# TGoldC/Motion-Planning-for-Autonomous-Driving-with-MPC

Hardware: AMD Instinct MI355X
Metric: MPC steps/sec (N=30, nx=6 nu=2) at batch=4096 (higher is better)
Workload: dtype f64; 1 GPU; N=30 nx=6 nu=2 bicycle lane-following, batch=4096/GPU, tol 1e-8; mode=converged, gpu=AMD Radeon Graphics

## Files before the change

motion-planning-for-autonomous-driving-with-mpc_amd/csrc/mpc_stamps.h:

```cpp
#pragma once
#include <algorithm>
#include <cstdarg>
#include <cstdio>
#include <string>
#include <vector>

namespace mpc {
constexpr int STAMP_SLOTS = 16;
#define MPC_STAMP(dbg, row, slot, pred) do { if ((dbg) && (pred)) (dbg)[(row) * STAMP_SLOTS + (slot)] = __builtin_amdgcn_s_memtime(); } while (0)

enum StageStamp { SB_ENTER, SB_ISSUED, SB_LOADED, SB_P1, SB_RED1, SB_LS, SB_UPDATE, SB_XCHG, SB_EVAL, SB_RED3, SB_END };
enum RicStamp { RT_BEGIN, RT_BWD_END, RT_FWD_END, RT_B15_WAIT, RT_B15_GO, RT_B15_END, RT_F15_WAIT, RT_F15_GO, RT_F15_END, RT_F0 };
enum PipeStamp { PW_TAKE = 11, PW_GOT, PW_BCAST, PW_DONE, PW_SIGNALLED,
                 PR_WAIT = 11, PR_SWEEP, PR_PUBLISHED };
enum WgStamp { WG_ROUND = 12, WG_RECORDS, WG_SWEPT, WG_ROUND_END };
enum StartStamp { PP_BOUNDS = 1, PP_DEFECTS, PP_SCAN1, PP_SCAN2, PP_SCAN3, PP_SUMS,
                  KS_BEGIN = 11, KS_ROWS, KS_STORED, KS_SAFE, KS_FENCED };

struct StampSpan { int from, to; const char* label; };
constexpr StampSpan START_SPANS[] = {
    {KS_BEGIN, KS_ROWS, "rows->LDS"}, {KS_ROWS, KS_STORED, "Z/REF stores"}, {KS_STORED, PP_BOUNDS, "bounds+a0"}, {PP_BOUNDS, PP_DEFECTS, "defects"}, {PP_DEFECTS, PP_SCAN1, "scan1"},
    {PP_SCAN1, PP_SCAN2, "tan+scan2"}, {PP_SCAN2, PP_SCAN3, "sincos+scan3"}, {PP_SCAN3, PP_SUMS, "ROLL+sums"}, {PP_SUMS, KS_SAFE, "decide"}, {KS_SAFE, KS_FENCED, "fence"},
    {KS_FENCED, SB_ENTER, "enter"}, {SB_ENTER, SB_XCHG, "init point+exchange"}, {SB_XCHG, SB_EVAL, "eval+assemble"}, {SB_EVAL, SB_RED3, "reduce"}, {SB_RED3, SB_END, "finish"}};
constexpr StampSpan WG_SPANS[] = {
    {WG_ROUND, WG_RECORDS, "records"}, {WG_RECORDS, WG_SWEPT, "sweeps"}, {WG_SWEPT, SB_ENTER, "enter"}, {SB_ENTER, SB_ISSUED, "load+premath"}, {SB_ISSUED, SB_LOADED, "or"}, {SB_LOADED, SB_P1, "P1"},
    {SB_P1, SB_RED1, "reduce1+ls-begin"}, {SB_RED1, SB_LS, "linesearch"}, {SB_LS, SB_UPDATE, "P3-update"}, {SB_UPDATE, SB_XCHG, "exchange"}, {SB_XCHG, SB_EVAL, "P4-eval"},
    {SB_EVAL, SB_RED3, "reduce3"}, {SB_RED3, SB_END, "P5"}, {SB_END, WG_ROUND_END, "drain"}};
constexpr StampSpan STAGE_SPANS[] = {
    {SB_ENTER, SB_ISSUED, "issue-loads"}, {SB_ISSUED, SB_LOADED, "wait+barrier"}, {SB_LOADED, SB_P1, "P1"}, {SB_P1, SB_RED1, "reduce1"}, {SB_RED1, SB_LS, "linesearch"},
    {SB_LS, SB_UPDATE, "P3-update"}, {SB_UPDATE, SB_XCHG, "exchange"}, {SB_XCHG, SB_EVAL, "P4-eval"}, {SB_EVAL, SB_RED3, "reduce3"}, {SB_RED3, SB_END, "P5"}};
constexpr StampSpan PIPE_STAGE_SPANS[] = {
    {PW_TAKE, PW_GOT, "dequeue"}, {PW_GOT, PW_BCAST, "acquire+bcast"}, {PW_BCAST, SB_ENTER, "enter"}, STAGE_SPANS[0], STAGE_SPANS[1], STAGE_SPANS[2], STAGE_SPANS[3], STAGE_SPANS[4], STAGE_SPANS[5],
    STAGE_SPANS[6], STAGE_SPANS[7], STAGE_SPANS[8], STAGE_SPANS[9], {SB_END, PW_DONE, "drain"}, {PW_DONE, PW_SIGNALLED, "signal"}};
constexpr StampSpan PIPE_RIC_SPANS[] = {
    {PR_WAIT, PR_SWEEP, "wait"}, {PR_SWEEP, RT_BWD_END, "backward"}, {RT_BWD_END, RT_FWD_END, "forward"}, {RT_FWD_END, PR_PUBLISHED, "publish"}, {RT_B15_WAIT, RT_B15_GO, "barrier"},
    {RT_B15_GO, RT_B15_END, "step"}, {RT_F15_WAIT, RT_F15_GO, "barrier"}, {RT_F15_GO, RT_F15_END, "step"}, {RT_BWD_END, RT_F0, "first forward stage"}};
constexpr StampSpan RIC_SPANS[] = {
    {RT_BEGIN, RT_BWD_END, "backward"}, {RT_BWD_END, RT_FWD_END, "forward"}, {RT_B15_WAIT, RT_B15_GO, "bwd barrier-wait"}, {RT_B15_GO, RT_B15_END, "compute"},
    {RT_F15_WAIT, RT_F15_GO, "fwd barrier-wait"}, {RT_F15_GO, RT_F15_END, "compute"}};

inline void appendf(std::string& s, const char* fmt, ...) {
    char buf[512];
    va_list ap;
    va_start(ap, fmt);
    vsnprintf(buf, sizeof buf, fmt, ap);
    va_end(ap);
    s += buf;
}
template <bool WRAP = false, size_t N, class Ran>
int span_sums(const unsigned long long* rows, int nrows, const StampSpan (&sp)[N], double (&acc)[N], Ran ran) {
    int cnt = 0;
    for (double& a : acc) a = 0.0;
    for (const unsigned long long* r = rows; r < rows + (size_t)nrows * STAMP_SLOTS; r += STAMP_SLOTS) {
        if (!ran(r)) continue;
        for (size_t q = 0; q < N; ++q) acc[q] += WRAP ? (double)(r[sp[q].to] - r[sp[q].from]) : (double)(long long)(r[sp[q].to] - r[sp[q].from]);
        ++cnt;
    }
    return cnt;
}
template <bool WRAP = false, size_t N, class Ran>
std::string span_means(const char* head, const unsigned long long* rows, int nrows, const StampSpan (&sp)[N], Ran ran) {
    double acc[N];
    const int cnt = span_sums<WRAP>(rows, nrows, sp, acc, ran);
    std::string s;
    appendf(s, head, cnt);
    for (size_t q = 0; q < N; ++q) appendf(s, " %s=%.0f", sp[q].label, cnt ? acc[q] / cnt : 0.0);
    return s;
}
inline std::string format_start_timing(const unsigned long long* rows, int nblk) {
    unsigned long long t0 = ~0ull, t1 = 0ull;
    for (int b = 0; b < nblk; ++b) { t0 = std::min(t0, rows[b * STAMP_SLOTS + KS_BEGIN]); t1 = std::max(t1, rows[b * STAMP_SLOTS + SB_END]); }
    std::string s = span_means("[mpcgpu k_start timing, shader-clock ticks, mean over %d workgroups]", rows, nblk, START_SPANS, [](const unsigned long long*) { return true; });
    appendf(s, "; first start to last end %.0f\n", (double)(t1 - t0));
    return s;
}
inline std::string format_wg_timing(const unsigned long long* rows, int nblk) {
    return span_means("[mpcgpu k_solve_wg timing, shader-clock ticks, third round of %d workgroups]", rows, nblk, WG_SPANS,
                      [](const unsigned long long* r) { return r[WG_ROUND_END] && r[SB_END]; }) + "\n";
}
inline std::string format_pipe_timing(const unsigned long long* rows, int n_wg) {
    auto stage = [](const unsigned long long* r) { return r[PW_SIGNALLED] && r[SB_END]; };
    std::string s = span_means("[mpcgpu pipeline timing, shader-clock ticks, last item of %d stage workers]", rows, n_wg, PIPE_STAGE_SPANS, stage);
    double ra[9];
    const int nr = span_sums(rows, n_wg, PIPE_RIC_SPANS, ra, [&](const unsigned long long* r) { return !stage(r) && r[PR_PUBLISHED] && r[RT_FWD_END]; });
    for (double& v : ra) v = nr ? v / nr : 0.0;
    appendf(s, "\n[last pass of %d Riccati workers] wait=%.0f backward=%.0f forward=%.0f publish=%.0f; stage 15 of the backward sweep: barrier=%.0f step=%.0f, of the forward sweep: barrier=%.0f step=%.0f, its first stage starts %.0f ticks after the backward sweep\n",
            nr, ra[0], ra[1], ra[2], ra[3], ra[4], ra[5], ra[6], ra[7], ra[8]);
    return s;
}
inline std::string format_stage_timing(const unsigned long long* rows, int nblk, int ntiles) {
    std::string s = span_means<true>("[mpcgpu stage timing, shader-clock ticks per block, mean over %d blocks]", rows, nblk, STAGE_SPANS,
                                     [](const unsigned long long* r) { return r[SB_END] != 0; }) + "\n";
    const unsigned long long* rr = rows + (size_t)8 * nblk;
    const int nt = std::min(ntiles, nblk / 2);
    auto ran = [](const unsigned long long* r) { return r[RT_FWD_END] != 0; };
    auto tile0 = [&](int q) { return (long long)(rr[RIC_SPANS[q].to] - rr[RIC_SPANS[q].from]); };
    if (nt > 0 && ran(rr))
        appendf(s, "[riccati stage 15 of tile 0] bwd barrier-wait=%lld compute=%lld | fwd barrier-wait=%lld compute=%lld\n", tile0(2), tile0(3), tile0(4), tile0(5));
    double ric[6];
    const int c2 = span_sums<true>(rr, nt, RIC_SPANS, ric, ran);
    appendf(s, "[mpcgpu riccati timing, ticks per workgroup, mean over %d] backward=%.0f forward=%.0f\n", c2, c2 ? ric[0] / c2 : 0.0, c2 ? ric[1] / c2 : 0.0);
    return s;
}
inline std::string format_wg_trace(const unsigned long long* hw, int n_wtrace) {
    unsigned long long t0 = ~0ull, t1 = 0ull;
    std::vector<int> live;
    for (int w = 0; w < n_wtrace; ++w) if (hw[4 * w + 2]) { t0 = std::min(t0, hw[4 * w]); t1 = std::max(t1, hw[4 * w + 1]); live.push_back(w); }
    std::string s;
    if (live.empty()) return s;
    std::sort(live.begin(), live.end(), [&](int a, int b) { return hw[4 * a + 1] > hw[4 * b + 1]; });
    int late = 0;
    double start_max = 0;
    for (int w : live) { const double st = (double)(hw[4 * w] - t0) * 1e-2; if (st > 5.0) ++late; start_max = std::max(start_max, st); }
    appendf(s, "[mpcgpu wg_trace] %d workgroups with work of %d; span %.1f us; %d of them start more than 5 us after the first (latest start %.1f us); the last to finish:\n",
            (int)live.size(), n_wtrace, (double)(t1 - t0) * 1e-2, late, start_max);
    for (size_t i = 0; i < live.size() && i < 12; ++i) {
        const int w = live[i];
        const double st = (double)(hw[4 * w] - t0) * 1e-2, en = (double)(hw[4 * w + 1] - t0) * 1e-2;
        const double tf = (double)((hw[4 * w + 3] >> 16) & 0xFFFFFFull) * 1e-2, tr1 = (double)((hw[4 * w + 3] >> 40) & 0xFFFFFFull) * 1e-2;
        appendf(s, "    workgroup %5d: start %6.1f us  end %6.1f us  rounds %2d  instance-rounds %2d  -> %.1f us per round; instances taken over after %.1f us, first round done after %.1f us, later rounds %.1f us each\n",
                w, st, en, (int)hw[4 * w + 2], (int)(hw[4 * w + 3] & 0xFFFFu), (en - st) / (double)hw[4 * w + 2], tf, tr1, hw[4 * w + 2] > 1 ? (en - st - tr1) / (double)(hw[4 * w + 2] - 1) : 0.0);
    }
    return s;
}

}
```

motion-planning-for-autonomous-driving-with-mpc_amd/csrc/mpcgpu.hip:

```cpp
#include <hip/hip_runtime.h>
#include <type_traits>

#include <algorithm>
#include <cctype>
#include <cstdio>
#include <cstdlib>
#include <cstring>
#include <new>
#include <string>
#include <vector>

#include "mpc_host_common.h"
#include "mpc_solve_plan.h"
#include "mpc_stamps.h"
#include "mpc_closed_loop.h"
#include "mpc_forces_qp.h"
#include "mpc_riccati_mfma.h"
#include "mpc_sens.h"
#include "mpc_loop_lin.h"

using namespace mpc;

namespace {

// ... 860 lines not shown
    }
    if (A.ho_list != nullptr && t < 64 && pipe_ld(abort_w) == 0u) {
        pipe_acquire();
        asm volatile("s_waitcnt vmcnt(0)" ::: "memory");
        for (;;) {
            uint32_t j = 0u;
            if (t == 0) j = pipe_add(X + PX_HO_TICKET, 1u);
            j = (uint32_t)__builtin_amdgcn_readfirstlane((int)j);
            if (j >= n_tiles_x) break;
            ho_lists(P, (j * n_xcd + xcd) * 64u + (uint32_t)t, A.ho_list, A.ctl + PIPE_HO, stage_done);
        }
    }
    if (t == 0) {
        unsigned long long* st = reinterpret_cast<unsigned long long*>(A.ctl + PIPE_STATS);
        atomicAdd(st + P64_STAGE_WAIT, waited);
        atomicAdd(st + P64_STAGE_BUSY, busy + wall_clock64());
        atomicAdd(st + P64_ITEMS, (unsigned long long)n_items);
        pipe_add(abort_w + PH_STAGE_WORKERS, 1u);
    }
#endif
}

struct PrestartFromWs {
    __device__ __forceinline__ double z(int, int, int) const { return 0.0; }
    __device__ __forceinline__ double ref0(int, int) const { return 0.0; }
};
template <int NX, class Src = PrestartFromWs> __device__ __forceinline__ void prestart_par_block(const PRef& P, const uint32_t b0, double* sm, const Src src = Src{});

template <int NX, bool OSTG = false>
__device__ __attribute__((noinline)) void wg_restart(const PRef& Pin, const int n_mult, const int n_z, const int stash_rows, const uint32_t b0, double* lds,
                                                     uint32_t* live_out, const bool carry, const bool from_xs, const bool keep_first, const bool first_tiled) {
    const PRef P = mpc_pref(static_cast<const Params&>(Pin), false);
    using D = Dim<NX>;
    const int t = threadIdx.x, N = P.N, bx = P.bx;
    struct { int b, k, mb, bl; } c;
    c.k = t / bx;
    c.bl = t & (bx - 1);
    c.mb = (int)blockIdx.x * bx;
    c.b = (int)b0 + c.bl;
    const bool valid = (c.k <= N) && (c.b < P.B);
    if (valid) {
        constexpr int NZ = D::NZ;
        double v[MPC_EV(NZ)];
        static_assert(2 * MPC_EV(NZ) <= D::NPK, "two iterates fit the cost-to-go rows of a stage");
        if (keep_first) {
            if (first_tiled) ws_load_rows<NZ>(MPC_ROWS(MPC_K(P.Z, NZ, 0, e)), v);
            else ws_load_rows<NZ>(MPC_ROWS(MPC_KI(P.MZ, NZ, 0, e)), v);
            ws_store_rows<NZ>(MPC_ROWS(MPC_K(P.PK, D::NPK, 0, MPC_EV(NZ) + e)), v);
            if (c.k == 0) MPC_S(P.SC, SC_E0S) = (double)MPC_S(P.SC, SC_E0);
        }
        if (carry) {
            ws_load_rows<NZ>(MPC_ROWS(MPC_KI(P.MZ, NZ, 0, e)), v);
            ws_store_rows<NZ>(MPC_ROWS(MPC_K(P.PK, D::NPK, 0, e)), v);
        }
        if (from_xs) {
            if (!carry) ws_load_rows<NZ>(MPC_ROWS(MPC_K(P.PK, D::NPK, 0, e)), v);
        } else {
            const size_t nw = (size_t)2 * N + (size_t)NX * (N + 1);
            const double* xr = P.x0 + (size_t)c.b * nw;
            v[0] = (c.k < N) ? MPC_GP(xr, 2 * c.k) : 0.0;
            v[1] = (c.k < N) ? MPC_GP(xr, 2 * c.k + 1) : 0.0;
#pragma unroll
            for (int i = 0; i < NX; ++i) v[2 + i] = MPC_GP(xr, 2 * N + NX * c.k + i);
        }
        ws_store_rows<NZ>(MPC_ROWS(MPC_K(P.Z, NZ, 0, e)), v);
    }
    asm volatile("s_waitcnt vmcnt(0)" ::: "memory");
    lds_barrier();
    __builtin_amdgcn_fence(__ATOMIC_ACQ_REL, "workgroup");
    asm volatile("s_waitcnt vmcnt(0)" ::: "memory");
    prestart_par_block<NX>(P, b0, lds);
    asm volatile("s_waitcnt vmcnt(0)" ::: "memory");
    lds_barrier();
    __builtin_amdgcn_fence(__ATOMIC_ACQ_REL, "workgroup");
    asm volatile("s_waitcnt vmcnt(0)" ::: "memory");
    stage_block<NX, true, 256, 0xFFu, NoStepWait, OSTG>(P, n_mult, n_z, stash_rows, b0, ~0ull, lds, false, live_out);
    asm volatile("s_waitcnt vmcnt(0)" ::: "memory");
    lds_barrier();
    __builtin_amdgcn_fence(__ATOMIC_ACQ_REL, "workgroup");
    asm volatile("s_waitcnt vmcnt(0)" ::: "memory");
}

template <int NX>
__device__ __attribute__((noinline)) void wg_restore_first(const PRef& Pin, const uint32_t b0, const int st0, const int it0) {
    const PRef P = mpc_pref(static_cast<const Params&>(Pin), false);
    using D = Dim<NX>;
    constexpr int NZ = D::NZ;
    const int t = threadIdx.x, bx = P.bx;
    struct { int b, k, mb, bl; } c;
    c.k = t / bx;
    c.bl = t & (bx - 1);
    c.mb = (int)blockIdx.x * bx;
    c.b = (int)b0 + c.bl;
    if (c.k <= P.N && c.b < P.B) {
        double v[MPC_EV(NZ)];
        ws_load_rows<NZ>(MPC_ROWS(MPC_K(P.PK, D::NPK, 0, MPC_EV(NZ) + e)), v);
        ws_store_rows<NZ>(MPC_ROWS(MPC_KI(P.MZ, NZ, 0, e)), v);
        ws_store_rows<NZ>(MPC_ROWS(MPC_K(P.Z, NZ, 0, e)), v);
        if (c.k == 0) {
            MPC_S(P.SC, SC_E0) = (double)MPC_S(P.SC, SC_E0S);
            MPC_S(P.ISC, IS_STATUS) = st0;
            MPC_S(P.ISC, IS_ITERS) = it0;
        }
    }
    asm volatile("s_waitcnt vmcnt(0)" ::: "memory");
    lds_barrier();
    __builtin_amdgcn_fence(__ATOMIC_ACQ_REL, "workgroup");
    asm volatile("s_waitcnt vmcnt(0)" ::: "memory");
}

struct WgRescue { double ol_raw, relax; int32_t on; };
constexpr int RESC_LEVELS = 8;
__device__ __forceinline__ double resc_fraction(int q) { return q == 2 || q == 7 ? 1.0 : q == 4 ? 0.4 : q == 5 ? 0.7 : q == 6 ? 0.9 : 0.0; }
__device__ __forceinline__ bool resc_last(int q) { return q == 2 || q == 7; }

#if defined(__HIP_DEVICE_COMPILE__)
typedef const __attribute__((address_space(4))) Params* mpc_kernarg_params;
__device__ __forceinline__ mpc_kernarg_params wg_kernarg() {
    mpc_kernarg_params kp = (mpc_kernarg_params)__builtin_amdgcn_kernarg_segment_ptr();
    asm volatile("" : "+s"(kp));
    return kp;
}
__device__ __forceinline__ EmitDst wg_emit_dst() {
    const mpc_kernarg_params kp = wg_kernarg();
    return EmitDst{kp->x_out, kp->status_out, kp->iters_out, kp->kkt_out, kp->fail_count};
}
#else
inline EmitDst wg_emit_dst() { return EmitDst{}; }
#endif
template <int NX, int VAR, bool RESC>
__device__ __forceinline__ void solve_wg_body(const Params& Pk, const int n_mult, const int n_z, const int stash_rows, uint32_t* stats, const uint32_t* skip_if,
                                              const WgRescue& resc, unsigned long long* wtrace, const int32_t* list, const uint32_t* list_n) {
    PRef P(Pk);
#if defined(__HIP_DEVICE_COMPILE__)
    const bool emit_exit = RESC && resc.on && Pk.emit != 0;
    if (RESC && emit_exit) P.emit = 0;
    extern __shared__ __attribute__((aligned(16))) double lds[];
    __shared__ uint32_t sh_mask;
    __shared__ int sh_next[2];
    if (skip_if != nullptr && *skip_if != 0u) return;
    const double tol0 = P.tol;
    bool fresh = true;
    using D = Dim<NX>;
    using RC = Rec<NX>;
    const int bx = P.bx, t = threadIdx.x, N = P.N;
    const int lane = t;
    const uint32_t b0 = (blockIdx.x + (uint32_t)P.tile0 * (64u / (uint32_t)bx)) * (uint32_t)bx;
    int ib0 = (int)b0 < P.B ? (int)b0 : -1, ib1 = (bx > 1 && (int)b0 + 1 < P.B) ? (int)b0 + 1 : -1;
    uint32_t in_mb = 0u;
    if (list != nullptr) {
        uint32_t cnt[HO_BUCKETS], n = 0u;
#pragma unroll
        for (int q = 0; q < (int)HO_BUCKETS; ++q) { cnt[q] = list_n[q]; n += cnt[q]; }
        auto entry = [&](uint32_t v) -> int {
            if (v >= n) return -1;
#pragma unroll
            for (int q = 0; q < (int)HO_BUCKETS; ++q) { if (v < cnt[q]) return list[(uint32_t)q * (uint32_t)P.Bp + v]; v -= cnt[q]; }
            return -1;
        };
        const uint32_t G = gridDim.x;
        ib0 = lds_uniform(entry(blockIdx.x));
        ib1 = bx > 1 ? lds_uniform(entry(2u * G - 1u - blockIdx.x)) : -1;
        if (ib0 < 0) return;
        in_mb = ((ib0 & HO_IN_MB) ? 1u : 0u) | ((ib1 >= 0 && (ib1 & HO_IN_MB)) ? 2u : 0u);
        ib0 &= ~HO_IN_MB;
        if (ib1 >= 0) ib1 &= ~HO_IN_MB;
    }
    struct { int b, k, mb, bl; } c;
    c.k = t / bx;
    c.bl = t & (bx - 1);
    c.mb = (int)blockIdx.x * bx;
    c.b = c.bl ? ib1 : ib0;
    const bool valid = (c.k <= N) && (c.b >= 0) && (c.b < P.B);
    const mpc_lds_ptr recs = (mpc_lds_ptr)(lds_ptr_t)lds + WgLds<NX>::PAD;
    const mpc_lds_ptr dump = (mpc_lds_ptr)(lds_ptr_t)lds;
    double* const lds_bnd = lds + WgLds<NX>::PAD + (size_t)RC::SIZE * ((N + 1) * bx);
    double* const lds_c0 = lds_bnd + 2 * (N + 1) * D::NZ;
    double* const lds_r0 = lds_c0 + 8 * bx;
    double* const lds_rn = lds_r0 + 8 * bx;
    double* const lds_scl = lds_rn + 64 * NX;
    bool bounds_ok = false;
    double dl0 = 0.0, dl1 = 0.0;
    WgIo io{0u, 0u, lds_c0, lds_rn, lds_r0, lds_scl, true, false};
    const MfmaWords lane_words = mfma_lane_load<NX>(lane);
    uint32_t rounds = 0, sweeps = 0, inst_rounds = 0, prev_mask = 0u;
    const unsigned long long t_begin = wtrace ? wall_clock64() : 0ull;
    unsigned long long t_fresh = 0ull, t_round1 = 0ull;
    if (RESC && resc.on && t == 0 && ib0 >= 0 && ib0 < P.B) MPC_UB(P.ISC, (uint32_t)IS_RLEV, ib0) = 0;
    for (;;) {
        if (rounds == 0u && t < 64) {
            const int bb = t ? ib1 : ib0;
            const bool run = t < bx && bb >= 0 && bb < P.B && (list != nullptr || (int32_t)MPC_UB(P.ISC, (uint32_t)IS_STATUS, bb >= 0 ? bb : 0) == ST_RUNNING);
            const unsigned long long mk = __ballot(run ? 1 : 0);
            if (t == 0) sh_mask = (uint32_t)mk;
        }
        lds_barrier();
        const uint32_t mask = lds_uniform(sh_mask);
        if (Pk.emit != 0 && !emit_exit) {
            const uint32_t gone = prev_mask & ~mask;
            if (gone != 0u && valid && ((gone >> c.bl) & 1u)) {
                double z[MPC_EV(D::NZ)];
                ws_load_rows<D::NZ>(MPC_ROWS(MPC_KI(P.MZ, D::NZ, 0, e)), z);
                int st = 0, it = 0;
                double e0 = 0.0;
                if (c.k == 0) { st = (int32_t)MPC_S(P.ISC, IS_STATUS); it = (int32_t)MPC_S(P.ISC, IS_ITERS); e0 = MPC_S(P.SC, SC_E0); }
                emit_row<NX>(wg_emit_dst(), N, c.b, c.k, z, st, it, e0);
            }
            prev_mask = mask;
        }
        if (mask == 0u) {
            if (!RESC || !resc.on) break;
            if (t == 0) {
                const int bb = ib0;
                int next = -1, carry = 0;
                if (bb >= 0 && bb < P.B) {
                    const int st = (int32_t)MPC_UB(P.ISC, (uint32_t)IS_STATUS, bb), it = (int32_t)MPC_UB(P.ISC, (uint32_t)IS_ITERS, bb);
                    const int lev = (int32_t)MPC_UB(P.ISC, (uint32_t)IS_RLEV, bb);
                    const int q = lev & 0xFF;
                    int has_xs = (lev >> 8) & 1, first = lev & ~0x1FF;
                    int acc = (q == 0 ? 0 : (int32_t)MPC_UB(P.ISC, (uint32_t)IS_ITACC, bb)) + it;
                    if (q == 0) {
                        if (st == 0 || st == -7) { next = 1; first = (st == -7 ? 0x200 : 0) | (it << 16); if (stats != nullptr) atomicAdd(stats + WGS_RESCUED, 1u); }
                    } else {
                        if (st == 1) { carry = 1; has_xs = 1; }
                        if (!resc_last(q)) next = q + 1;
                        else if (st != 1 && q == 2) { next = 3; has_xs = 0; acc = first >> 16; }
                    }
                    if (next >= 0) {
                        MPC_UB(P.ISC, (uint32_t)IS_RLEV, bb) = next | (has_xs << 8) | first;
                        MPC_UB(P.ISC, (uint32_t)IS_ITACC, bb) = acc;
                        next |= has_xs << 8;
                    } else if (q != 0) {
                        if (st == 1) MPC_UB(P.ISC, (uint32_t)IS_ITERS, bb) = acc;
                        else next = -2 - ((first >> 9) & 1) - 2 * (first >> 16);
                    }
                }
                sh_next[0] = next;
                sh_next[1] = carry;
            }
            lds_barrier();
            const int nx_lev = lds_uniform(sh_next[0]), carry = lds_uniform(sh_next[1]);
            lds_barrier();
            if (nx_lev <= -2) {
                const int code = -2 - nx_lev;
                const PRef Pc = P;
                wg_restore_first<NX>(Pc, (uint32_t)ib0, (code & 1) ? -7 : 0, code >> 1);
            }
            if (nx_lev < 0) break;
            const int q = nx_lev & 0xFF;
            const bool from_xs = (nx_lev >> 8) != 0;
            {
                const double lo = resc_fraction(q) * resc.ol_raw;
                P.ol = lo - resc.relax * fmax(1.0, fabs(lo));
                P.tol = resc_last(q) ? tol0 : fmax(tol0, 1e-4);
            }
            {
                const PRef Pc = P;
                if (VAR == 2 || Pc.per_inst_obst != OBST_PER_STAGE) wg_restart<NX>(Pc, n_mult, n_z, stash_rows, (uint32_t)ib0, lds, &sh_mask, carry != 0, from_xs, q == 1, rounds == 0u);
                else wg_restart<NX, true>(Pc, n_mult, n_z, stash_rows, (uint32_t)ib0, lds, &sh_mask, carry != 0, from_xs, q == 1, rounds == 0u);
            }
            fresh = true;
            bounds_ok = false;
            io.have = false;
            continue;
        }
        ++rounds;
        inst_rounds += (uint32_t)__popc(mask);
        MPC_STAMP(P.DBG, blockIdx.x, WG_ROUND, t == 0 && rounds == 3u);
        const bool by_pipe = !RESC && valid && ((in_mb >> c.bl) & 1u) != 0u;
        if (fresh && valid && !by_pipe) {
            auto move = [&](auto cnt, auto from, auto to) {
                constexpr int CNT = decltype(cnt)::value;
                double v[MPC_EV(CNT)];
                ws_load_rows<CNT>(from, v);
                ws_store_rows<CNT>(to, v);
            };
            constexpr int NZ = D::NZ;
            move(std::integral_constant<int, NZ>{}, MPC_ROWS(MPC_K(P.Z, NZ, 0, e)), MPC_ROWS(MPC_KI(P.MZ, NZ, 0, e)));
            move(std::integral_constant<int, NZ>{}, MPC_ROWS(MPC_K(P.ZL, NZ, 0, e)), MPC_ROWS(MPC_KI(P.MZL, NZ, 0, e)));
            move(std::integral_constant<int, NZ>{}, MPC_ROWS(MPC_K(P.ZU, NZ, 0, e)), MPC_ROWS(MPC_KI(P.MZU, NZ, 0, e)));
            move(std::integral_constant<int, 4>{}, MPC_ROWS(MPC_K(P.SO, 3, 0, e)), MPC_ROWS(MPC_KI(P.MSO, 3, 0, e)));
            move(std::integral_constant<int, 4>{}, MPC_ROWS(MPC_K(P.NUO, 3, 0, e)), MPC_ROWS(MPC_KI(P.MNUO, 3, 0, e)));
            move(std::integral_constant<int, 4>{}, MPC_ROWS(MPC_K(P.ZLO, 3, 0, e)), MPC_ROWS(MPC_KI(P.MZLO, 3, 0, e)));
            move(std::integral_constant<int, 4>{}, MPC_ROWS(MPC_K(P.ZUO, 3, 0, e)), MPC_ROWS(MPC_KI(P.MZUO, 3, 0, e)));
            move(std::integral_constant<int, NX>{}, MPC_ROWS(MPC_K(P.LAM, NX, 0, e)), MPC_ROWS(MPC_KI(P.MLAM, NX, 0, e)));
        }
        if (fresh) {
            asm volatile("s_waitcnt vmcnt(0)" ::: "memory");
            __builtin_amdgcn_fence(__ATOMIC_ACQ_REL, "workgroup");
            asm volatile("s_waitcnt vmcnt(0)" ::: "memory");
        }
        const bool whole = fresh, tiled = fresh && !by_pipe;
        auto build_records = [&]() {
            if (valid && ((mask >> (t & (bx - 1))) & 1u)) {
                double blk[MPC_EV(D::NBLK)];
                if (tiled) ws_load_rows<D::NBLK>(MPC_ROWS(MPC_K(P.BLK, D::NBLK, 0, e)), blk);
                else ws_load_rows<D::NBLK>(MPC_ROWS(MPC_KI(P.MBLK, D::NBLK, 0, e)), blk);
                double hx0 = 0.0, hx1 = 0.0;
                if (c.k == 0) { hx0 = MPC_S(P.SC, SC_HUX0); hx1 = MPC_S(P.SC, SC_HUX1); }
                const mpc_lds_ptr r = recs + ((t & (bx - 1)) * (N + 1) + c.k) * RC::SIZE;
#pragma unroll
                for (int i = 0; i < D::NBLK; ++i) {
                    const bool kept = i < D::B_RUU || (i >= D::B_CN && i < D::B_CN + NX);
                    if (whole || !kept) r[RC::slot(i)] = (i >= D::B_CN && i < D::B_CN + NX) ? -blk[i] : blk[i];
                }
                r[RC::ZERO] = 0.0;
                r[RC::ONE] = 1.0;
                r[RC::DT] = P.dt;
                r[RC::HX] = hx0;
                r[RC::HX + 1] = hx1;
            }
        };
        if (fresh) {
            build_records();
            const int a0 = ib0 >= 0 ? ib0 : 0, a1 = ib1 >= 0 ? ib1 : a0;
            dl0 = lds_uniform((double)MPC_UB(P.SC, (uint32_t)SC_DLAST, a0));
            dl1 = lds_uniform((double)MPC_UB(P.SC, (uint32_t)SC_DLAST, a1));
            io.ill = ((int32_t)MPC_UB(P.ISC, (uint32_t)IS_ILL, a0) != 0 ? 1u : 0u) | ((bx > 1 && (int32_t)MPC_UB(P.ISC, (uint32_t)IS_ILL, a1) != 0) ? 2u : 0u);
            if (valid && c.k == 0) {
#pragma unroll
                for (int i = 0; i < NX; ++i) lds_c0[(t & (bx - 1)) * 8 + i] = MPC_S(P.SC, SC_C0 + i);
                double* q = lds_scl + c.bl * WgScl::SIZE;
                q[WgScl::MU] = MPC_S(P.SC, SC_MU); q[WgScl::TAU] = MPC_S(P.SC, SC_TAU); q[WgScl::DF] = MPC_S(P.SC, SC_DF); q[WgScl::THETA] = MPC_S(P.SC, SC_THETA);
                q[WgScl::FCOST] = MPC_S(P.SC, SC_FCOST); q[WgScl::LOGSUM] = MPC_S(P.SC, SC_LOGSUM); q[WgScl::THMAX] = MPC_S(P.SC, SC_THMAX);
                q[WgScl::THMIN] = MPC_S(P.SC, SC_THMIN); q[WgScl::A0LB] = MPC_S(P.SC, SC_A0LB); q[WgScl::A0UB] = MPC_S(P.SC, SC_A0UB);
                q[WgScl::STATUS] = (double)(int32_t)MPC_S(P.ISC, IS_STATUS); q[WgScl::NFILT] = (double)(int32_t)MPC_S(P.ISC, IS_NFILT);
                q[WgScl::ITERS] = (double)(int32_t)MPC_S(P.ISC, IS_ITERS); q[WgScl::CONV] = (double)(int32_t)MPC_S(P.ISC, IS_CONV);
                q[WgScl::FROW] = (double)(int32_t)MPC_S(P.ISC, IS_FROW); q[WgScl::HAVETH0] = (double)(int32_t)MPC_S(P.ISC, IS_HAVETH0);
            }
            {
                const bool f0 = ib0 >= 0 && t < 2 * FILTER_MAX, f1 = bx > 1 && ib1 >= 0 && t < 2 * FILTER_MAX;
                const double v0 = f0 ? (double)ws_ref3(P, P.FILT, 0u, (uint32_t)ib0, mpc_prow((uint32_t)t)) : 0.0;
                const double v1 = f1 ? (double)ws_ref3(P, P.FILT, 0u, (uint32_t)ib1, mpc_prow((uint32_t)t)) : 0.0;
                if (f0) lds_scl[WgScl::FILT + t] = v0;
                if (f1) lds_scl[WgScl::SIZE + WgScl::FILT + t] = v1;
            }
        }
        if (!bounds_ok) {
            const int nb = (N + 1) * D::NZ;
            fill_bounds<8>(P, lds_bnd, nb, t, 64);
            bounds_ok = true;
        }
        lds_barrier();
        if (wtrace != nullptr && fresh && t_fresh == 0ull) t_fresh = wall_clock64() - t_begin;
        fresh = false;
        MPC_STAMP(P.DBG, blockIdx.x, WG_RECORDS, t == 0 && rounds == 3u);
        MfmaWords lw = lane_words;
        asm volatile("" : "+v"(lw.w[0]), "+v"(lw.w[1]), "+v"(lw.w[2]), "+v"(lw.w[3]));
        MfmaLane<NX> m;
        mfma_lane_setup<NX>(m, lw, P.dt);
        constexpr uint32_t SVM = VAR == 2 ? REF_VM : 0xFFu;
        {
            auto inst_of = [&](int g, MfmaInst& in, double& x0) {
                in.inst = (uint32_t)(g ? ib1 : ib0);
                in.delta_last = g ? dl1 : dl0;
                in.sym_hint = ((io.ill >> g) & 1u) != 0u;
                x0 = 0.0;
                if ((lane & 3) == 0) {
                    if (m.Rb < NX) x0 = -lds_c0[g * 8 + m.Rb];
                    else if (m.Rb == 7) x0 = 1.0;
                }
            };
            io.fail = 0u;
            auto finish = [&](int g, bool ok, double delta) {
                const int bb = g ? ib1 : ib0;
                if (ok) { if (delta > 0.0) { if (g) dl1 = lds_uniform(delta); else dl0 = lds_uniform(delta); } }
                else io.fail |= 1u << g;
                if (lane != 0) return;
                if (ok) {
                    if (delta > 0.0) MPC_UB(P.SC, (uint32_t)SC_DLAST, bb) = delta;
                    MPC_UB(P.SC, (uint32_t)SC_DELTA, bb) = delta;
                } else {
                    MPC_UB(P.ISC, (uint32_t)IS_STATUS, bb) = -7;
                }
            };
            auto rebuild = [&]() { lds_barrier(); build_records(); lds_barrier(); };
            const int g0 = __builtin_ctz(mask);
            const bool two = (mask & (mask - 1u)) != 0u;
            const int g1 = two ? 1 : g0;
            MfmaInst in[2];
            double x0[2], delta[2];
            bool ok[2];
            inst_of(g0, in[0], x0[0]);
            inst_of(g1, in[1], x0[1]);
            const mpc_lds_ptr rec[2] = {recs + g0 * (N + 1) * RC::SIZE, recs + g1 * (N + 1) * RC::SIZE};
            typedef const MfmaInst (&In1)[1];
            typedef const mpc_lds_ptr (&Rec1)[1];
            typedef double (&D1)[1];
            typedef const double (&CD1)[1];
            typedef bool (&B1)[1];
            typedef const bool (&CB1)[1];
            if (two) mfma_backward<NX, 2>(P, m, in, rec, lane, dump, delta, ok, sweeps, rebuild);
            else mfma_backward<NX, 1>(P, m, reinterpret_cast<In1>(in), reinterpret_cast<Rec1>(rec), lane, dump, reinterpret_cast<D1>(delta), reinterpret_cast<B1>(ok), sweeps, rebuild);
            if (t == 0) sh_mask = 0u;
            wg_stage<NX, SVM>(P, ib0, ib1, lds_bnd, recs, n_mult, n_z, rounds == 3u, &sh_mask, io, [&]() {
                if (two) mfma_forward<NX, 2>(P, m, in, rec, lane, dump, x0, ok);
                else mfma_forward<NX, 1>(P, m, reinterpret_cast<In1>(in), reinterpret_cast<Rec1>(rec), lane, dump, reinterpret_cast<CD1>(x0), reinterpret_cast<CB1>(ok));
                finish(g0, ok[0], delta[0]);
                if (two) finish(g1, ok[1], delta[1]);
                lds_barrier();
                MPC_STAMP(P.DBG, blockIdx.x, WG_SWEPT, t == 0 && rounds == 3u);
            });
            io.have = true;
        }
        asm volatile("s_waitcnt vmcnt(0)" ::: "memory");
        lds_barrier();
        __builtin_amdgcn_fence(__ATOMIC_ACQ_REL, "workgroup");
        asm volatile("s_waitcnt vmcnt(0)" ::: "memory");
        MPC_STAMP(P.DBG, blockIdx.x, WG_ROUND_END, t == 0 && rounds == 3u);
        if (wtrace != nullptr && rounds == 1u) t_round1 = wall_clock64() - t_begin;
    }
    if (rounds > 0u && valid && !Pk.emit) {
        double v[D::NZ];
        ws_load_rows<D::NZ>(MPC_ROWS(MPC_KI(P.MZ, D::NZ, 0, e)), v);
        ws_store_rows<D::NZ>(MPC_ROWS(MPC_K(P.Z, D::NZ, 0, e)), v);
    }
    if (RESC && emit_exit && valid) {
        double z[MPC_EV(D::NZ)];
        if (rounds > 0u) ws_load_rows<D::NZ>(MPC_ROWS(MPC_KI(P.MZ, D::NZ, 0, e)), z);
        else ws_load_rows<D::NZ>(MPC_ROWS(MPC_K(P.Z, D::NZ, 0, e)), z);
        int st = 0, it = 0;
        double e0 = 0.0;
        if (c.k == 0) { st = (int32_t)MPC_S(P.ISC, IS_STATUS); it = (int32_t)MPC_S(P.ISC, IS_ITERS); e0 = MPC_S(P.SC, SC_E0); if (st == ST_RUNNING) st = 0; }
        emit_row<NX>(wg_emit_dst(), N, c.b, c.k, z, st, it, e0);
    }
    if (wtrace != nullptr && t == 0) {
        wtrace[blockIdx.x * 4 + 0] = t_begin;
        wtrace[blockIdx.x * 4 + 1] = wall_clock64();
        wtrace[blockIdx.x * 4 + 2] = rounds;
        wtrace[blockIdx.x * 4 + 3] = (unsigned long long)(inst_rounds & 0xFFFFu) | ((t_fresh & 0xFFFFFFull) << 16) | ((t_round1 & 0xFFFFFFull) << 40);
    }
    if (stats != nullptr && t == 0) {
        atomicMax(stats + WGS_ROUNDS_MAX, rounds);
        atomicAdd(stats + WGS_ROUNDS, rounds);
        atomicAdd(stats + WGS_SWEEPS, sweeps);
        atomicAdd(stats + WGS_INST_ROUNDS, inst_rounds);
    }
#endif
}
template <int NX, int VAR, bool RESC = false>
__global__ void __launch_bounds__(256) k_solve_wg(const Params Pk, const int n_mult, const int n_z, const int stash_rows, uint32_t* stats, const uint32_t* skip_if,
                                                                   const WgRescue resc, unsigned long long* wtrace, const int32_t* list, const uint32_t* list_n) {
    solve_wg_body<NX, VAR, RESC>(Pk, n_mult, n_z, stash_rows, stats, skip_if, resc, wtrace, list, list_n);
#if defined(__HIP_DEVICE_COMPILE__)
    if (threadIdx.x < 64) {
        const mpc_kernarg_params kp = wg_kernarg();
        uint32_t* const ctl = kp->fin_ctl;
        if (ctl == nullptr) return;
        uint32_t tk = 0u;
        if (threadIdx.x == 0) {
            asm volatile("s_waitcnt vmcnt(0)" ::: "memory");
            tk = __hip_atomic_fetch_add(ctl + PH_FIN_TICKET, 1u, __ATOMIC_RELAXED, __HIP_MEMORY_SCOPE_AGENT);
        }
        tk = (uint32_t)__builtin_amdgcn_readfirstlane((int)tk);
        if (tk == gridDim.x - 1u && threadIdx.x < PH_WORDS) {
            const uint32_t v = __hip_atomic_load(ctl + threadIdx.x, __ATOMIC_RELAXED, __HIP_MEMORY_SCOPE_AGENT);
            __hip_atomic_store(kp->fin_host + threadIdx.x, v, __ATOMIC_RELAXED, __HIP_MEMORY_SCOPE_SYSTEM);
        }
    }
#endif
}

template <int NX, class Src>
__device__ __forceinline__ void prestart_par_block(const PRef& P, const uint32_t b0, double* sm, const Src src) {
    constexpr bool WS = std::is_same<Src, PrestartFromWs>::value;
    constexpr int NZ = NX + 2;
    const int N = P.N, S = N + 1, bx = P.bx, t = threadIdx.x, bl = t & (bx - 1);
    const int nb = S * NZ, SB = S * bx;
    double* LBt = sm;
    double* UBt = LBt + nb;
    double* XR = UBt + nb;
    double* DR = XR + NX * SB;
    double* DG = DR + NX * SB;
    double* IN = DG + NX * SB;
    double* A0 = IN + 2 * SB;
    double* PLt = A0 + 4 * bx;
    double* PHt = PLt + nb;
    struct { int b, k; } c;
    c.k = t / bx;
    c.b = (int)b0 + bl;
    const bool valid = c.k <= N && c.b < P.B;
    const uint32_t bb = (uint32_t)c.b;
    for (int q0 = 0; q0 < nb; q0 += 2 * (int)blockDim.x) {
        double lo[2], hi[2];
#pragma unroll
        for (int j = 0; j < 2; ++j) { const int q = q0 + j * (int)blockDim.x + t; lo[j] = q < nb ? (double)MPC_GP(P.LB, q) : 0.0; hi[j] = q < nb ? (double)MPC_GP(P.UB, q) : 0.0; }
#pragma unroll
        for (int j = 0; j < 2; ++j) {
            const int q = q0 + j * (int)blockDim.x + t;
            if (q < nb) { double L, H; push_limits(lo[j], hi[j], L, H); LBt[q] = lo[j]; UBt[q] = hi[j]; PLt[q] = L; PHt[q] = H; }
        }
    }
    double a0lb = 0.0, a0ub = 0.0;
    int frow = 1;
    if (valid && c.k == 0) {
// ... 2917 lines not shown
```

Measured before the change: 5.780 million MPC steps/s.

## Hoist instance take-over loads before the round loop and batch them per phase

Moves the fresh-instance work (moving iterate rows to the multi-buffer, loading records, scalars, filter and bounds into LDS) out of the main round loop into a take_over routine that runs once before the loop for the non-rescue path. Each phase issues all of its global loads first, waits once, then writes to LDS, so load latency overlaps instead of being serialised. The list lookup now computes indices first and issues both list loads together. The trace printer also gains median/max summary lines. The risk is higher register pressure from holding the batched loads, and an ordering change in the rescue path.

Result: no change. 5.782 million MPC steps/s (median of 2 runs) (+0.0%).

```diff
diff --git a/motion-planning-for-autonomous-driving-with-mpc_amd/csrc/mpc_stamps.h b/motion-planning-for-autonomous-driving-with-mpc_amd/csrc/mpc_stamps.h
--- a/motion-planning-for-autonomous-driving-with-mpc_amd/csrc/mpc_stamps.h
+++ b/motion-planning-for-autonomous-driving-with-mpc_amd/csrc/mpc_stamps.h
@@ -114,6 +114,13 @@
     for (int w : live) { const double st = (double)(hw[4 * w] - t0) * 1e-2; if (st > 5.0) ++late; start_max = std::max(start_max, st); }
     appendf(s, "[mpcgpu wg_trace] %d workgroups with work of %d; span %.1f us; %d of them start more than 5 us after the first (latest start %.1f us); the last to finish:\n",
             (int)live.size(), n_wtrace, (double)(t1 - t0) * 1e-2, late, start_max);
+    std::vector<double> tfs, tr1s;
+    for (int w : live) {
+        const unsigned long long f = (hw[4 * w + 3] >> 16) & 0xFFFFFFull, r1 = (hw[4 * w + 3] >> 40) & 0xFFFFFFull;
+        if (f) tfs.push_back((double)f * 1e-2);
+        if (r1) tr1s.push_back((double)r1 * 1e-2);
+    }
+    auto median = [](std::vector<double>& v) { std::sort(v.begin(), v.end()); return v[v.size() / 2]; };
     for (size_t i = 0; i < live.size() && i < 12; ++i) {
         const int w = live[i];
         const double st = (double)(hw[4 * w] - t0) * 1e-2, en = (double)(hw[4 * w + 1] - t0) * 1e-2;
@@ -121,6 +128,11 @@
         appendf(s, "    workgroup %5d: start %6.1f us  end %6.1f us  rounds %2d  instance-rounds %2d  -> %.1f us per round; instances taken over after %.1f us, first round done after %.1f us, later rounds %.1f us each\n",
                 w, st, en, (int)hw[4 * w + 2], (int)(hw[4 * w + 3] & 0xFFFFu), (en - st) / (double)hw[4 * w + 2], tf, tr1, hw[4 * w + 2] > 1 ? (en - st - tr1) / (double)(hw[4 * w + 2] - 1) : 0.0);
     }
+    if (!tfs.empty() && !tr1s.empty()) {
+        const double fm = median(tfs), rm = median(tr1s);
+        appendf(s, "    over %d workgroups: instances taken over after median %.1f us, max %.1f us; first round done after median %.1f us, max %.1f us\n",
+                (int)tfs.size(), fm, tfs.back(), rm, tr1s.back());
+    }
     return s;
 }
 
diff --git a/motion-planning-for-autonomous-driving-with-mpc_amd/csrc/mpcgpu.hip b/motion-planning-for-autonomous-driving-with-mpc_amd/csrc/mpcgpu.hip
--- a/motion-planning-for-autonomous-driving-with-mpc_amd/csrc/mpcgpu.hip
+++ b/motion-planning-for-autonomous-driving-with-mpc_amd/csrc/mpcgpu.hip
@@ -1036,15 +1036,17 @@
         uint32_t cnt[HO_BUCKETS], n = 0u;
 #pragma unroll
         for (int q = 0; q < (int)HO_BUCKETS; ++q) { cnt[q] = list_n[q]; n += cnt[q]; }
-        auto entry = [&](uint32_t v) -> int {
-            if (v >= n) return -1;
-#pragma unroll
-            for (int q = 0; q < (int)HO_BUCKETS; ++q) { if (v < cnt[q]) return list[(uint32_t)q * (uint32_t)P.Bp + v]; v -= cnt[q]; }
-            return -1;
+        auto where = [&](uint32_t v) -> uint32_t {
+            if (v >= n) return ~0u;
+#pragma unroll
+            for (int q = 0; q < (int)HO_BUCKETS; ++q) { if (v < cnt[q]) return (uint32_t)q * (uint32_t)P.Bp + v; v -= cnt[q]; }
+            return ~0u;
         };
         const uint32_t G = gridDim.x;
-        ib0 = lds_uniform(entry(blockIdx.x));
-        ib1 = bx > 1 ? lds_uniform(entry(2u * G - 1u - blockIdx.x)) : -1;
+        const uint32_t w0 = where(blockIdx.x), w1 = bx > 1 ? where(2u * G - 1u - blockIdx.x) : ~0u;
+        const int e0 = list[w0 != ~0u ? w0 : 0u], e1 = list[w1 != ~0u ? w1 : 0u];
+        ib0 = lds_uniform(w0 != ~0u ? e0 : -1);
+        ib1 = lds_uniform(w1 != ~0u ? e1 : -1);
         if (ib0 < 0) return;
         in_mb = ((ib0 & HO_IN_MB) ? 1u : 0u) | ((ib1 >= 0 && (ib1 & HO_IN_MB)) ? 2u : 0u);
         ib0 &= ~HO_IN_MB;
@@ -1063,7 +1065,6 @@
     double* const lds_r0 = lds_c0 + 8 * bx;
     double* const lds_rn = lds_r0 + 8 * bx;
     double* const lds_scl = lds_rn + 64 * NX;
-    bool bounds_ok = false;
     double dl0 = 0.0, dl1 = 0.0;
     WgIo io{0u, 0u, lds_c0, lds_rn, lds_r0, lds_scl, true, false};
     const MfmaWords lane_words = mfma_lane_load<NX>(lane);
@@ -1071,13 +1072,143 @@
     const unsigned long long t_begin = wtrace ? wall_clock64() : 0ull;
     unsigned long long t_fresh = 0ull, t_round1 = 0ull;
     if (RESC && resc.on && t == 0 && ib0 >= 0 && ib0 < P.B) MPC_UB(P.ISC, (uint32_t)IS_RLEV, ib0) = 0;
-    for (;;) {
-        if (rounds == 0u && t < 64) {
+    auto first_mask = [&]() {
+        if (t < 64) {
             const int bb = t ? ib1 : ib0;
             const bool run = t < bx && bb >= 0 && bb < P.B && (list != nullptr || (int32_t)MPC_UB(P.ISC, (uint32_t)IS_STATUS, bb >= 0 ? bb : 0) == ST_RUNNING);
             const unsigned long long mk = __ballot(run ? 1 : 0);
             if (t == 0) sh_mask = (uint32_t)mk;
         }
+    };
+    const bool by_pipe = !RESC && valid && ((in_mb >> c.bl) & 1u) != 0u;
+    auto load_records = [&](const bool tiled, double* blk, double& hx0, double& hx1) {
+        if (tiled) ws_load_rows<D::NBLK>(MPC_ROWS(MPC_K(P.BLK, D::NBLK, 0, e)), blk);
+        else ws_load_rows<D::NBLK>(MPC_ROWS(MPC_KI(P.MBLK, D::NBLK, 0, e)), blk);
+        hx0 = 0.0; hx1 = 0.0;
+        if (c.k == 0) { hx0 = MPC_S(P.SC, SC_HUX0); hx1 = MPC_S(P.SC, SC_HUX1); }
+    };
+    auto store_records = [&](const bool whole, const double* blk, const double hx0, const double hx1) {
+        const mpc_lds_ptr r = recs + ((t & (bx - 1)) * (N + 1) + c.k) * RC::SIZE;
+#pragma unroll
+        for (int i = 0; i < D::NBLK; ++i) {
+            const bool kept = i < D::B_RUU || (i >= D::B_CN && i < D::B_CN + NX);
+            if (whole || !kept) r[RC::slot(i)] = (i >= D::B_CN && i < D::B_CN + NX) ? -blk[i] : blk[i];
+        }
+        r[RC::ZERO] = 0.0;
+        r[RC::ONE] = 1.0;
+        r[RC::DT] = P.dt;
+        r[RC::HX] = hx0;
+        r[RC::HX + 1] = hx1;
+    };
+    auto rec_on = [&](const uint32_t mask) { return valid && ((mask >> (t & (bx - 1))) & 1u); };
+    constexpr int TK_MOVE_A = 1, TK_MOVE_B = 16, TK_REC = 2, TK_SCL = 4, TK_BND = 8;
+    auto take_over = [&](auto parts, const uint32_t mask) {
+        constexpr int PARTS = decltype(parts)::value;
+        const bool on = (PARTS & TK_REC) && rec_on(mask);
+        const bool scl = (PARTS & TK_SCL) && valid && c.k == 0;
+        constexpr int NZ = D::NZ;
+        constexpr int BJ = 16;
+        static_assert(NZ <= 8, "the bounds table of one wavefront's instances is one trip of BJ loads per lane");
+        const int nb = (N + 1) * NZ;
+        auto move_rows = [&]() {
+            if (!valid || by_pipe) return;
+            if (PARTS & TK_MOVE_A) {
+                double mz[MPC_EV(NZ)], mzl[MPC_EV(NZ)], mzu[MPC_EV(NZ)];
+                ws_load_rows<NZ>(MPC_ROWS(MPC_K(P.Z, NZ, 0, e)), mz);
+                ws_load_rows<NZ>(MPC_ROWS(MPC_K(P.ZL, NZ, 0, e)), mzl);
+                ws_load_rows<NZ>(MPC_ROWS(MPC_K(P.ZU, NZ, 0, e)), mzu);
+                ws_store_rows<NZ>(MPC_ROWS(MPC_KI(P.MZ, NZ, 0, e)), mz);
+                ws_store_rows<NZ>(MPC_ROWS(MPC_KI(P.MZL, NZ, 0, e)), mzl);
+                ws_store_rows<NZ>(MPC_ROWS(MPC_KI(P.MZU, NZ, 0, e)), mzu);
+            }
+            if (PARTS & TK_MOVE_B) {
+                double mso[4], mnuo[4], mzlo[4], mzuo[4], mlam[MPC_EV(NX)];
+                ws_load_rows<4>(MPC_ROWS(MPC_K(P.SO, 3, 0, e)), mso);
+                ws_load_rows<4>(MPC_ROWS(MPC_K(P.NUO, 3, 0, e)), mnuo);
+                ws_load_rows<4>(MPC_ROWS(MPC_K(P.ZLO, 3, 0, e)), mzlo);
+                ws_load_rows<4>(MPC_ROWS(MPC_K(P.ZUO, 3, 0, e)), mzuo);
+                ws_load_rows<NX>(MPC_ROWS(MPC_K(P.LAM, NX, 0, e)), mlam);
+                ws_store_rows<4>(MPC_ROWS(MPC_KI(P.MSO, 3, 0, e)), mso);
+                ws_store_rows<4>(MPC_ROWS(MPC_KI(P.MNUO, 3, 0, e)), mnuo);
+                ws_store_rows<4>(MPC_ROWS(MPC_KI(P.MZLO, 3, 0, e)), mzlo);
+                ws_store_rows<4>(MPC_ROWS(MPC_KI(P.MZUO, 3, 0, e)), mzuo);
+                ws_store_rows<NX>(MPC_ROWS(MPC_KI(P.MLAM, NX, 0, e)), mlam);
+            }
+        };
+        if (PARTS & (TK_MOVE_A | TK_MOVE_B)) move_rows();
+        double blk[MPC_EV(D::NBLK)], hx0 = 0.0, hx1 = 0.0;
+        if (on) load_records(!by_pipe, blk, hx0, hx1);
+        const int a0 = ib0 >= 0 ? ib0 : 0, a1 = ib1 >= 0 ? ib1 : a0;
+        double vdl0 = 0.0, vdl1 = 0.0;
+        int32_t ill0 = 0, ill1 = 0;
+        if (PARTS & TK_SCL) {
+            vdl0 = MPC_UB(P.SC, (uint32_t)SC_DLAST, a0); vdl1 = MPC_UB(P.SC, (uint32_t)SC_DLAST, a1);
+            ill0 = MPC_UB(P.ISC, (uint32_t)IS_ILL, a0); ill1 = MPC_UB(P.ISC, (uint32_t)IS_ILL, a1);
+        }
+        constexpr int SC_ROW[10] = {SC_MU, SC_TAU, SC_DF, SC_THETA, SC_FCOST, SC_LOGSUM, SC_THMAX, SC_THMIN, SC_A0LB, SC_A0UB};
+        constexpr int IS_ROW[6] = {IS_STATUS, IS_NFILT, IS_ITERS, IS_CONV, IS_FROW, IS_HAVETH0};
+        static_assert(WgScl::MU == 0 && WgScl::A0UB == 9 && WgScl::STATUS == 10 && WgScl::HAVETH0 == 15, "the two row lists above follow WgScl");
+        double c0v[NX], scv[10];
+        int32_t isv[6];
+        if (scl) {
+#pragma unroll
+            for (int i = 0; i < NX; ++i) c0v[i] = MPC_S(P.SC, SC_C0 + i);
+#pragma unroll
+            for (int i = 0; i < 10; ++i) scv[i] = MPC_S(P.SC, SC_ROW[i]);
+#pragma unroll
+            for (int i = 0; i < 6; ++i) isv[i] = MPC_S(P.ISC, IS_ROW[i]);
+        }
+        const bool f0 = (PARTS & TK_SCL) && ib0 >= 0 && t < 2 * FILTER_MAX, f1 = (PARTS & TK_SCL) && bx > 1 && ib1 >= 0 && t < 2 * FILTER_MAX;
+        const double fv0 = f0 ? (double)ws_ref3(P, P.FILT, 0u, (uint32_t)ib0, mpc_prow((uint32_t)t)) : 0.0;
+        const double fv1 = f1 ? (double)ws_ref3(P, P.FILT, 0u, (uint32_t)ib1, mpc_prow((uint32_t)t)) : 0.0;
+        double bv[BJ];
+#pragma unroll
+        for (int j = 0; j < BJ; ++j) { const int q = j * 64 + t; bv[j] = !(PARTS & TK_BND) ? 0.0 : q < nb ? (double)MPC_GP(P.LB, q) : q < 2 * nb ? (double)MPC_GP(P.UB, q - nb) : 0.0; }
+        asm volatile("s_waitcnt vmcnt(0)" ::: "memory");
+        __builtin_amdgcn_fence(__ATOMIC_ACQ_REL, "workgroup");
+        asm volatile("s_waitcnt vmcnt(0)" ::: "memory");
+        asm volatile("" : "+v"(vdl0), "+v"(vdl1), "+v"(ill0), "+v"(ill1));
+#pragma unroll
+        for (int i = 0; i < 6; ++i) asm volatile("" : "+v"(isv[i]));
+        if (on) store_records(true, blk, hx0, hx1);
+        if (PARTS & TK_SCL) {
+            dl0 = lds_uniform(vdl0);
+            dl1 = lds_uniform(vdl1);
+            io.ill = (ill0 != 0 ? 1u : 0u) | ((bx > 1 && ill1 != 0) ? 2u : 0u);
+        }
+        if (scl) {
+#pragma unroll
+            for (int i = 0; i < NX; ++i) lds_c0[(t & (bx - 1)) * 8 + i] = c0v[i];
+            double* q = lds_scl + c.bl * WgScl::SIZE;
+#pragma unroll
+            for (int i = 0; i < 10; ++i) q[i] = scv[i];
+#pragma unroll
+            for (int i = 0; i < 6; ++i) q[WgScl::STATUS + i] = (double)isv[i];
+        }
+        if (f0) lds_scl[WgScl::FILT + t] = fv0;
+        if (f1) lds_scl[WgScl::SIZE + WgScl::FILT + t] = fv1;
+#pragma unroll
+        for (int j = 0; j < BJ; ++j) { const int q = j * 64 + t; if ((PARTS & TK_BND) && q < 2 * nb) lds_bnd[q] = bv[j]; }
+    };
+    auto take_over_all = [&](const uint32_t mask) {
+        take_over(std::integral_constant<int, TK_MOVE_A>{}, mask);
+        take_over(std::integral_constant<int, TK_MOVE_B>{}, mask);
+        if (RESC) {
+            take_over(std::integral_constant<int, TK_SCL>{}, mask);
+            take_over(std::integral_constant<int, TK_BND>{}, mask);
+        } else {
+            take_over(std::integral_constant<int, TK_SCL | TK_BND>{}, mask);
+        }
+        take_over(std::integral_constant<int, TK_REC>{}, mask);
+    };
+    if (!RESC) {
+        first_mask();
+        lds_barrier();
+        const uint32_t mask = lds_uniform(sh_mask);
+        if (mask != 0u) take_over_all(mask);
+    }
+    for (;;) {
+        if (RESC && rounds == 0u) first_mask();
         lds_barrier();
         const uint32_t mask = lds_uniform(sh_mask);
         if (Pk.emit != 0 && !emit_exit) {
@@ -1144,87 +1275,20 @@
                 else wg_restart<NX, true>(Pc, n_mult, n_z, stash_rows, (uint32_t)ib0, lds, &sh_mask, carry != 0, from_xs, q == 1, rounds == 0u);
             }
             fresh = true;
-            bounds_ok = false;
             io.have = false;
             continue;
         }
         ++rounds;
         inst_rounds += (uint32_t)__popc(mask);
         MPC_STAMP(P.DBG, blockIdx.x, WG_ROUND, t == 0 && rounds == 3u);
-        const bool by_pipe = !RESC && valid && ((in_mb >> c.bl) & 1u) != 0u;
-        if (fresh && valid && !by_pipe) {
-            auto move = [&](auto cnt, auto from, auto to) {
-                constexpr int CNT = decltype(cnt)::value;
-                double v[MPC_EV(CNT)];
-                ws_load_rows<CNT>(from, v);
-                ws_store_rows<CNT>(to, v);
-            };
-            constexpr int NZ = D::NZ;
-            move(std::integral_constant<int, NZ>{}, MPC_ROWS(MPC_K(P.Z, NZ, 0, e)), MPC_ROWS(MPC_KI(P.MZ, NZ, 0, e)));
-            move(std::integral_constant<int, NZ>{}, MPC_ROWS(MPC_K(P.ZL, NZ, 0, e)), MPC_ROWS(MPC_KI(P.MZL, NZ, 0, e)));
-            move(std::integral_constant<int, NZ>{}, MPC_ROWS(MPC_K(P.ZU, NZ, 0, e)), MPC_ROWS(MPC_KI(P.MZU, NZ, 0, e)));
-            move(std::integral_constant<int, 4>{}, MPC_ROWS(MPC_K(P.SO, 3, 0, e)), MPC_ROWS(MPC_KI(P.MSO, 3, 0, e)));
-            move(std::integral_constant<int, 4>{}, MPC_ROWS(MPC_K(P.NUO, 3, 0, e)), MPC_ROWS(MPC_KI(P.MNUO, 3, 0, e)));
-            move(std::integral_constant<int, 4>{}, MPC_ROWS(MPC_K(P.ZLO, 3, 0, e)), MPC_ROWS(MPC_KI(P.MZLO, 3, 0, e)));
-            move(std::integral_constant<int, 4>{}, MPC_ROWS(MPC_K(P.ZUO, 3, 0, e)), MPC_ROWS(MPC_KI(P.MZUO, 3, 0, e)));
-            move(std::integral_constant<int, NX>{}, MPC_ROWS(MPC_K(P.LAM, NX, 0, e)), MPC_ROWS(MPC_KI(P.MLAM, NX, 0, e)));
-        }
-        if (fresh) {
-            asm volatile("s_waitcnt vmcnt(0)" ::: "memory");
-            __builtin_amdgcn_fence(__ATOMIC_ACQ_REL, "workgroup");
-            asm volatile("s_waitcnt vmcnt(0)" ::: "memory");
-        }
-        const bool whole = fresh, tiled = fresh && !by_pipe;
+        if (RESC && fresh) take_over_all(mask);
         auto build_records = [&]() {
-            if (valid && ((mask >> (t & (bx - 1))) & 1u)) {
-                double blk[MPC_EV(D::NBLK)];
-                if (tiled) ws_load_rows<D::NBLK>(MPC_ROWS(MPC_K(P.BLK, D::NBLK, 0, e)), blk);
-                else ws_load_rows<D::NBLK>(MPC_ROWS(MPC_KI(P.MBLK, D::NBLK, 0, e)), blk);
-                double hx0 = 0.0, hx1 = 0.0;
-                if (c.k == 0) { hx0 = MPC_S(P.SC, SC_HUX0); hx1 = MPC_S(P.SC, SC_HUX1); }
-                const mpc_lds_ptr r = recs + ((t & (bx - 1)) * (N + 1) + c.k) * RC::SIZE;
-#pragma unroll
-                for (int i = 0; i < D::NBLK; ++i) {
-                    const bool kept = i < D::B_RUU || (i >= D::B_CN && i < D::B_CN + NX);
-                    if (whole || !kept) r[RC::slot(i)] = (i >= D::B_CN && i < D::B_CN + NX) ? -blk[i] : blk[i];
-                }
-                r[RC::ZERO] = 0.0;
-                r[RC::ONE] = 1.0;
-                r[RC::DT] = P.dt;
-                r[RC::HX] = hx0;
-                r[RC::HX + 1] = hx1;
+            if (rec_on(mask)) {
+                double blk[MPC_EV(D::NBLK)], hx0, hx1;
+                load_records(false, blk, hx0, hx1);
+                store_records(false, blk, hx0, hx1);
             }
         };
-        if (fresh) {
-            build_records();
-            const int a0 = ib0 >= 0 ? ib0 : 0, a1 = ib1 >= 0 ? ib1 : a0;
-            dl0 = lds_uniform((double)MPC_UB(P.SC, (uint32_t)SC_DLAST, a0));
-            dl1 = lds_uniform((double)MPC_UB(P.SC, (uint32_t)SC_DLAST, a1));
-            io.ill = ((int32_t)MPC_UB(P.ISC, (uint32_t)IS_ILL, a0) != 0 ? 1u : 0u) | ((bx > 1 && (int32_t)MPC_UB(P.ISC, (uint32_t)IS_ILL, a1) != 0) ? 2u : 0u);
-            if (valid && c.k == 0) {
-#pragma unroll
-                for (int i = 0; i < NX; ++i) lds_c0[(t & (bx - 1)) * 8 + i] = MPC_S(P.SC, SC_C0 + i);
-                double* q = lds_scl + c.bl * WgScl::SIZE;
-                q[WgScl::MU] = MPC_S(P.SC, SC_MU); q[WgScl::TAU] = MPC_S(P.SC, SC_TAU); q[WgScl::DF] = MPC_S(P.SC, SC_DF); q[WgScl::THETA] = MPC_S(P.SC, SC_THETA);
-                q[WgScl::FCOST] = MPC_S(P.SC, SC_FCOST); q[WgScl::LOGSUM] = MPC_S(P.SC, SC_LOGSUM); q[WgScl::THMAX] = MPC_S(P.SC, SC_THMAX);
-                q[WgScl::THMIN] = MPC_S(P.SC, SC_THMIN); q[WgScl::A0LB] = MPC_S(P.SC, SC_A0LB); q[WgScl::A0UB] = MPC_S(P.SC, SC_A0UB);
-                q[WgScl::STATUS] = (double)(int32_t)MPC_S(P.ISC, IS_STATUS); q[WgScl::NFILT] = (double)(int32_t)MPC_S(P.ISC, IS_NFILT);
-                q[WgScl::ITERS] = (double)(int32_t)MPC_S(P.ISC, IS_ITERS); q[WgScl::CONV] = (double)(int32_t)MPC_S(P.ISC, IS_CONV);
-                q[WgScl::FROW] = (double)(int32_t)MPC_S(P.ISC, IS_FROW); q[WgScl::HAVETH0] = (double)(int32_t)MPC_S(P.ISC, IS_HAVETH0);
-            }
-            {
-                const bool f0 = ib0 >= 0 && t < 2 * FILTER_MAX, f1 = bx > 1 && ib1 >= 0 && t < 2 * FILTER_MAX;
-                const double v0 = f0 ? (double)ws_ref3(P, P.FILT, 0u, (uint32_t)ib0, mpc_prow((uint32_t)t)) : 0.0;
-                const double v1 = f1 ? (double)ws_ref3(P, P.FILT, 0u, (uint32_t)ib1, mpc_prow((uint32_t)t)) : 0.0;
-                if (f0) lds_scl[WgScl::FILT + t] = v0;
-                if (f1) lds_scl[WgScl::SIZE + WgScl::FILT + t] = v1;
-            }
-        }
-        if (!bounds_ok) {
-            const int nb = (N + 1) * D::NZ;
-            fill_bounds<8>(P, lds_bnd, nb, t, 64);
-            bounds_ok = true;
-        }
         lds_barrier();
         if (wtrace != nullptr && fresh && t_fresh == 0ull) t_fresh = wall_clock64() - t_begin;
         fresh = false;
```
